# kerry-he/fsae-mpc

Hardware: AMD Instinct MI355X
Metric: QP solves/sec (batched LTV-MPC, N=40 nx=5 nu=2 fp64) (higher is better)
Workload: dtype f64

## Files before the change

### fsae-mpc_amd/_lib.py

```python
import ctypes as C
import os

_HERE = os.path.dirname(os.path.abspath(__file__))
LIB_PATH = os.environ.get("FSAEMPC_LIB") or os.path.join(_HERE, "lib", "libfsaempc.so")

EXPORTS = [
    "fsaempc_qp_default_opts", "fsaempc_qp_workspace_bytes", "fsaempc_qp_solve_batch_device", "fsaempc_qp_solve_batch",
    "fsaempc_ltv_nx", "fsaempc_ltv_nV", "fsaempc_ltv_nC", "fsaempc_ltv_build_qp_batch_device",
    "fsaempc_ltv_workspace_bytes", "fsaempc_ltv_step_batch_device", "fsaempc_ltv_step_batch_device_aux", "fsaempc_last_error", "fsaempc_selftest_mfma", "fsaempc_selftest_lane_reduce", "fsaempc_selftest_diag_factor", "fsaempc_selftest_initial_point",
    "fsaempc_debug_set_dump", "fsaempc_qp_solve_batch_device_aux", "fsaempc_qp_set_timing", "fsaempc_qp_get_timing", "fsaempc_ltv_get_timing",
    "fsaempc_seq_init", "fsaempc_seq_hotstart", "fsaempc_seq_hotstart_matrices", "fsaempc_seq_equality", "fsaempc_seq_cleanup",
    "fsaempc_obtain_reference_batch_device", "fsaempc_reference_live_batch_device",
    "fsaempc_cl_pre_batch_device", "fsaempc_cl_plant_batch_device", "fsaempc_cl_accept_batch_device",
    "fsaempc_track_from_csv", "fsaempc_track_from_points", "fsaempc_track_free", "fsaempc_track_save", "fsaempc_track_load", "fsaempc_track_last_error",
    "fsaempc_nlp_build_qp_batch_device", "fsaempc_sqp_default_opts", "fsaempc_sqp_workspace_bytes", "fsaempc_sqp_batch_device",
    "fsaempc_sqp_get_timing", "fsaempc_qp_vjp_workspace_bytes", "fsaempc_qp_vjp_batch_device",
    "fsaempc_ltv_affine_maps_batch_device", "fsaempc_ltv_step_batch_device_lambda", "fsaempc_ltv_step_vjp_workspace_bytes",
    "fsaempc_ltv_step_vjp_batch_device",
    "fsaempc_ltv_default_params", "fsaempc_ltv_build_qp_batch_device_p", "fsaempc_ltv_step_batch_device_p",
    "fsaempc_nlp_build_qp_batch_device_p", "fsaempc_sqp_batch_device_p", "fsaempc_cl_plant_batch_device_p",
    "fsaempc_ltv_blocked_nV", "fsaempc_ltv_build_qp_batch_device_b", "fsaempc_ltv_workspace_bytes_b", "fsaempc_ltv_step_batch_device_b",
    "fsaempc_qp_workspace_bytes_s", "fsaempc_qp_solve_batch_device_s", "fsaempc_qp_layout",
    "fsaempc_plan_profile_batch_device", "fsaempc_plan_reference_batch_device", "fsaempc_cl_pre_plan_batch_device",
    "fsaempc_raceline_build_qp_device", "fsaempc_plan_line_profile_batch_device", "fsaempc_plan_raceline_workspace_bytes",
# ... 345 lines not shown
```

### fsae-mpc_amd/csrc/capi_qp.hip

```cpp
#include <mutex>
#include <vector>
#include "capi_common.h"
#include "qp_solver.h"
#include "qp_sens.h"

namespace capi __attribute__((visibility("hidden"))) {
__thread char g_err[512] = "";
std::atomic<double*> g_dump{nullptr}; std::atomic<int> g_dump_stage{0};
std::atomic<bool> g_timing{false}; hipEvent_t g_ev[3] = {nullptr, nullptr, nullptr};
hipEvent_t g_evf[2] = {nullptr, nullptr};
hipEvent_t g_evs[5] = {nullptr, nullptr, nullptr, nullptr, nullptr};
double g_sqp_ms[4] = {0, 0, 0, 0};
}
using namespace capi;

extern "C" {

const char* fsaempc_last_error(void) { return g_err; }

void fsaempc_qp_default_opts(fsaempc_qp_opts* o) {
  if (!o) return;
  o->tol = 1e-8; o->tol_loose = 1e-6; o->tol_x = 1e-7; o->inf_bound = 1e9; o->max_iter = 100; o->polish = 1;
}

// ... 313 lines not shown
  return 0;
}

static int selftest(int (*test)(char* msg, int msglen)) {
  int cnt = 0;
  hipError_t e = hipGetDeviceCount(&cnt);
  if (e != hipSuccess || cnt == 0) return fail(FSAEMPC_ERR_NODEVICE, "no HIP device");
  char msg[256] = "";
  int bad = test(msg, sizeof(msg));
  if (bad != 0) snprintf(g_err, sizeof(g_err), "%s", msg);
  return bad;
}
int fsaempc_selftest_mfma(void) { return selftest(qp_selftest_mfma); }
int fsaempc_selftest_lane_reduce(void) { return selftest(qp_selftest_lane_reduce); }
int fsaempc_selftest_diag_factor(void) { return selftest(qp_selftest_diag_factor); }
int fsaempc_selftest_initial_point(void) { return selftest(qp_selftest_initial_point); }

int fsaempc_debug_set_dump(double* out, int stage) { g_dump.store(out); g_dump_stage.store(stage); return 0; }

int fsaempc_qp_set_timing(int enable) {
  if (enable && !g_ev[0]) {
    for (hipEvent_t& ev : g_ev) if (int rc = launched(hipEventCreate(&ev), "hipEventCreate")) return rc;
    for (hipEvent_t& ev : g_evf) if (int rc = launched(hipEventCreate(&ev), "hipEventCreate")) return rc;
    for (hipEvent_t& ev : g_evs) if (int rc = launched(hipEventCreate(&ev), "hipEventCreate")) return rc;
  }
  g_timing.store(enable != 0);
  return 0;
}

int fsaempc_ltv_get_timing(double* build_ms, double* prep_ms, double* solve_ms, double* post_ms) {
// ... 31 lines not shown
```

### fsae-mpc_amd/csrc/qp_probe.h

```cpp
#pragma once
#include "qp_solve_kernel.h"

template <int T, int NB> __global__ __launch_bounds__(64) void syrk_probe_kernel(QpParams P, int reps) {
  const int b = blockIdx.x;
  extern __shared__ double lds[];
  Ctx k;
  ctx_setup<T>(k, P, b, lds);
  const QpSolveLds L = qp_solve_lds(T, NB, P.d.np);
  double* MB = lds + L.vecs;
  k.ring = MB + L.border + L.tiles; k.cof = k.ring + L.ring;
  for (int js = 0; js < k.JT; ++js) {
    const int ix = js * 64 + k.lane;
    rowp(k, R_D)[ix] = 1.0; rowp(k, R_W1)[ix] = 0.5; rowp(k, R_W2)[ix] = 0.25; rowp(k, R_W3)[ix] = 2.0;
  }
  __syncthreads();
  v4d acc[Tri<T>::NT];
  acc_init<T>(k, acc);
  const unsigned long long t0 = __builtin_amdgcn_s_memtime();
  for (int r = 0; r < reps; ++r) {
    Stream<T> st;
    st.open(k);
    pass_syrk<T, NB>(k, st, acc, vecp(k, V_P1), vecp(k, V_P2), vecp(k, V_P3), MB);
    st.close();
    __syncthreads();
  }
  const unsigned long long t1 = __builtin_amdgcn_s_memtime();
  double cs = 0;
#pragma unroll
  for (int i = 0; i < Tri<T>::NT; ++i) cs += acc[i][0] + acc[i][1] + acc[i][2] + acc[i][3];
  cs = wave_sum(cs);
  if (k.lane == 0) { P.dump[b] = (double)(t1 - t0) / reps; P.dump[gridDim.x + b] = cs; }
}

__global__ __launch_bounds__(64) void overlap_probe_kernel(double* out, int reps) {
  const double x = 1.0 + 1e-9 * threadIdx.x, y = 1e-12 * (threadIdx.x + 1);
  v4d acc[8]; double f[8];
#pragma unroll
  for (int i = 0; i < 8; ++i) { acc[i] = v4d{0.0, 0.0, 0.0, 0.0}; f[i] = 1.0 + i; }
  __builtin_amdgcn_sched_barrier(0);
  const unsigned long long t0 = __builtin_amdgcn_s_memtime();
  for (int r = 0; r < reps; ++r) {
#pragma unroll
    for (int i = 0; i < 16; ++i) acc[i & 7] = __builtin_amdgcn_mfma_f64_16x16x4f64(x, y, acc[i & 7], 0, 0, 0);
    __builtin_amdgcn_sched_barrier(0);
  }
  const unsigned long long t1 = __builtin_amdgcn_s_memtime();
  for (int r = 0; r < reps; ++r) {
#pragma unroll
    for (int i = 0; i < 32; ++i) f[i & 7] = fma(f[i & 7], x, y);
    __builtin_amdgcn_sched_barrier(0);
  }
  const unsigned long long t2 = __builtin_amdgcn_s_memtime();
  for (int r = 0; r < reps; ++r) {
#pragma unroll
    for (int i = 0; i < 16; ++i) {
      acc[i & 7] = __builtin_amdgcn_mfma_f64_16x16x4f64(x, y, acc[i & 7], 0, 0, 0);
      f[(2 * i) & 7] = fma(f[(2 * i) & 7], x, y); f[(2 * i + 1) & 7] = fma(f[(2 * i + 1) & 7], x, y);
    }
// ... 26 lines not shown
  for (int r = 0; r < reps; ++r) {
    acc_init<T>(k, acc);
#pragma unroll
    for (int K = 0; K < T; ++K) {
#pragma unroll
      for (int p = 0; p < 4; ++p) if (k.q + 4 * p == k.c) acc[Tri<T>::idx(K, K)][p] += 20.0;
    }
    for (int i = k.lane; i < 16 * T; i += 64) RV[i] = 1.0 + (i & 15);
    __syncthreads();
    __builtin_amdgcn_sched_barrier(0);
    unsigned long long t0 = __builtin_amdgcn_s_memtime();
    reg_factor<T, 1>(k, acc, YL, 1e-30);
    __builtin_amdgcn_sched_barrier(0);
    unsigned long long t1 = __builtin_amdgcn_s_memtime();
    tt[0] += t1 - t0;
    v4d Yk, none = {0.0, 0.0, 0.0, 0.0};
#pragma unroll
    for (int K = 0; K < T; ++K) {
#pragma unroll
      for (int p = 0; p < 4; ++p) { Yk[p] = (k.q + 4 * p == k.c) ? 1.0 : 0.0; if (k.q + 4 * p == k.c) acc[Tri<T>::idx(K, K)][p] += 30.0; }
      diag_factor<DiagForm<T, 1>::form>(k, acc[Tri<T>::idx(K, K)], Yk, none, 1e-30);
      cs += Yk[0];
    }
    __builtin_amdgcn_sched_barrier(0);
    unsigned long long t2 = __builtin_amdgcn_s_memtime();
    tt[1] += t2 - t1;
#pragma unroll
    for (int K = 0; K < T; ++K) { tile_store(k, YL + K * 272, acc[Tri<T>::idx(K, K)]); __syncthreads(); acc[Tri<T>::idx(K, K)] = tile_load_t(k, YL + K * 272); }
    __builtin_amdgcn_sched_barrier(0);
    unsigned long long t3 = __builtin_amdgcn_s_memtime();
    tt[2] += t3 - t2;
    double y[T][4];
    vec_forward<T, true>(k, acc, YL, RV, y);
    WAVE_SYNC();
    vec_backward<T, true>(k, acc, YL, y, RV);
    WAVE_SYNC();
// ... 10 lines not shown
```

### fsae-mpc_amd/csrc/qp_selftest.h

```cpp
#pragma once
#include <stdlib.h>
#include <stdio.h>
#include "qp_solve_kernel.h"

namespace {

__global__ void mfma_selftest_kernel(const double* Am, const double* Bm, double* Cm) {
  const int lane = threadIdx.x;
  const double a = Am[(lane & 15) * 4 + (lane >> 4)];
  const double bb = Bm[(lane >> 4) * 16 + (lane & 15)];
  v4d c = {0, 0, 0, 0};
  c = __builtin_amdgcn_mfma_f64_16x16x4f64(a, bb, c, 0, 0, 0);
#pragma unroll
  for (int p = 0; p < 4; ++p) Cm[((lane >> 4) + 4 * p) * 16 + (lane & 15)] = c[p];
}

DEVINL bool same_bits(double a, double b) { return __double_as_longlong(a) == __double_as_longlong(b) || (a != a && b != b); }
template <class OP> DEVINL double lds_grp16(double* sh, int lane, double v) {
  const int src[4] = {lane ^ 1, lane ^ 2, (lane & ~7) | (7 - (lane & 7)), (lane & ~15) | (15 - (lane & 15))};
#pragma unroll
  for (int s = 0; s < 4; ++s) {
    sh[lane] = v; __syncthreads();
    const double o = sh[src[s]]; __syncthreads();
    v = OP::f(v, o);
// ... 72 lines not shown
      double a[4] = {x[4], x[5], x[6], x[7]};
      wave_sum(a);
      int nb = 0;
#pragma unroll
      for (int i = 0; i < 4; ++i) nb += same_bits(a[i], wave_sum_zf(x[4 + i])) ? 0 : 1;
      if (nb && first < 0) first = 100 * 65;
      bad += nb;
    }
    if (bad != before && first_round < 0) first_round = r;
  }
  if (bad) {
    if (atomicAdd(&out[0], bad) == 0) { out[1] = first; out[2] = first_round; out[3] = lane; }
  }
}

template <int FORM> DEVINL int diag_factor_bad_vs_old(const Ctx& k, const v4d& U0, const v4d& R0, double floor_abs, const v4d& Uo, const v4d& Yo, const v4d& Ro, int bo) {
  v4d U = U0, R = R0, Y;
#pragma unroll
  for (int p = 0; p < 4; ++p) Y[p] = (k.q + 4 * p == k.c) ? 1.0 : 0.0;
  const int b = diag_factor<FORM>(k, U, Y, R, floor_abs);
  int bad = (b != bo) ? 1 : 0;
#pragma unroll
  for (int p = 0; p < 4; ++p)
    bad += (__double_as_longlong(U[p]) != __double_as_longlong(Uo[p])) + (__double_as_longlong(Y[p]) != __double_as_longlong(Yo[p])) +
           (__double_as_longlong(R[p]) != __double_as_longlong(Ro[p]));
  return bad;
}
__global__ __launch_bounds__(64) void diag_factor_selftest_kernel(const double* __restrict__ in, int ntiles, double floor_abs, int* __restrict__ out) {
  Ctx k = {};
  k.lane = threadIdx.x; k.c = k.lane & 15; k.q = k.lane >> 4;
  int bad = 0, first = -1, form = 0;
  for (int t = 0; t < ntiles; ++t) {
    v4d U0, R0, Uo, Ro, Yo;
#pragma unroll
    for (int p = 0; p < 4; ++p) {
      U0[p] = in[(size_t)t * 512 + (k.q + 4 * p) * 16 + k.c];
      R0[p] = in[(size_t)t * 512 + 256 + (k.q + 4 * p) * 16 + k.c];
      Yo[p] = (k.q + 4 * p == k.c) ? 1.0 : 0.0;
    }
    Uo = U0; Ro = R0;
    const int bo = diag_factor<0>(k, Uo, Yo, Ro, floor_abs);
    const int b1 = diag_factor_bad_vs_old<1>(k, U0, R0, floor_abs, Uo, Yo, Ro, bo);
    const int b2 = diag_factor_bad_vs_old<2>(k, U0, R0, floor_abs, Uo, Yo, Ro, bo);
    if ((b1 | b2) && first < 0) { first = t; form = b1 ? 1 : 2; }
    bad += b1 + b2;
  }
  if (bad) {
    if (atomicAdd(&out[0], bad) == 0) { out[1] = first; out[2] = form; out[3] = k.lane; }
  }
}

template <int T, int NB> __global__ __launch_bounds__(64) void initial_point_selftest_kernel(QpParams P, int* __restrict__ out) {
  extern __shared__ double lds[];
  Ctx k;
  (void)ctx_setup<T>(k, P, 0, lds);
  const QpSolveLds L = qp_solve_lds(T, NB, P.d.np);
  k.ring = lds + L.vecs + L.border + L.tiles;
  k.cof = k.ring + L.ring;
  const int lane = k.lane, J = k.J, JT = k.JT;
  double* Xv = vecp(k, V_X); double* P3o = vecp(k, V_P1); double* P3n = vecp(k, V_P3);
  double* W3 = rowp(k, R_W3); double* Vo = rowp(k, R_VA); double* Vn = rowp(k, R_V);
  const double* Lb = rowp(k, R_L); const double* Ub = rowp(k, R_U);
  Stream<T> st;
// ... 127 lines not shown
  }
  double* d = 0; int* dout = 0; int hout[4] = {0, 0, 0, 0};
  if (hipMalloc(&d, sizeof(double) * ntiles * 512) != hipSuccess || hipMalloc(&dout, sizeof(hout)) != hipSuccess) { free(h); if (d) (void)hipFree(d); return -1; }
  (void)hipMemcpy(d, h, sizeof(double) * ntiles * 512, hipMemcpyHostToDevice);
  (void)hipMemset(dout, 0, sizeof(hout));
  free(h);
  hipLaunchKernelGGL(diag_factor_selftest_kernel, dim3(1), dim3(64), 0, 0, d, ntiles, floor_abs, dout);
  hipError_t e = hipDeviceSynchronize();
  if (e == hipSuccess) e = hipMemcpy(hout, dout, sizeof(hout), hipMemcpyDeviceToHost);
  (void)hipFree(d); (void)hipFree(dout);
  if (e != hipSuccess) { snprintf(msg, msglen, "diag_factor selftest: %s", hipGetErrorString(e)); return -1; }
  if (hout[0]) snprintf(msg, msglen, "diag_factor forms: %d mismatches with the former form, first: tile %d form %d lane %d", hout[0], hout[1], hout[2], hout[3]);
  return hout[0];
}

template <int T, int NB> static hipError_t initial_point_launch(const QpParams& P, int* dout) {
  hipError_t e = hipFuncSetAttribute(reinterpret_cast<const void*>(&initial_point_selftest_kernel<T, NB>), hipFuncAttributeMaxDynamicSharedMemorySize, (int)P.d.lds_solve);
  if (e != hipSuccess) return e;
  hipLaunchKernelGGL((initial_point_selftest_kernel<T, NB>), dim3(1), dim3(64), P.d.lds_solve, 0, P, dout);
  return hipGetLastError();
}
static int initial_point_shape(int nV, int nC, char* msg, int msglen) {
  QpDims d;
  qp_make_dims(nV, nC, &d);
  const int nb = d.nb, ncu = nV - nb;
  const double inf = 1e20;
  const size_t nH = (size_t)nV * nV, nA = (size_t)nC * nV, nin = nH + nA + 3 * (size_t)nV + 2 * (size_t)nC;
  double* h = (double*)calloc(nin, sizeof(double));
  if (!h) return -1;
  double *H = h, *A = H + nH, *g = A + nA, *lb = g + nV, *ub = lb + nV, *lbA = ub + nV, *ubA = lbA + nC;
// ... 76 lines not shown
```

### fsae-mpc_amd/csrc/qp_solve_kernel.h

```cpp
#pragma once
#include "qp_solver.h"
#include "qp_lane.h"
#include "qp_rules.h"

#ifndef QP_SOLVE_PAIR
#define QP_SOLVE_PAIR 0
#endif
#ifndef QP_DIAG_FLAT
#define QP_DIAG_FLAT 1
#endif
#ifndef QP_SYRK_INTERLEAVE
#define QP_SYRK_INTERLEAVE 0
#endif
#ifndef QP_STARTUP_ATW
#define QP_STARTUP_ATW 0
#endif
#ifndef QP_SWEEP_BATCH
#define QP_SWEEP_BATCH 6
#endif

namespace {

template <int T> struct Tri {
  static constexpr int NT = T * (T + 1) / 2;
// ... 446 lines not shown
  v4d Z;
#pragma unroll
  for (int p = 0; p < 4; ++p) Z[p] = slot[(k.q + 4 * p) * 17 + k.c];
  return Z;
}
DEVINL v4d tile_load_t(const Ctx& k, const double* slot) {
  v4d Z;
#pragma unroll
  for (int p = 0; p < 4; ++p) Z[p] = slot[k.c * 17 + k.q + 4 * p];
  return Z;
}

DEVINL double on_lanes(unsigned long long mask, double v, double otherwise) {
  return __builtin_amdgcn_inverse_ballot_w64(mask) ? v : otherwise;
}
template <int FORM> DEVINL int diag_factor(const Ctx& k, v4d& Ud, v4d& Yk, v4d& rk, double floor_abs) {
  constexpr bool FLAT = FORM >= 1;
  int bad = 0;
#pragma unroll
  for (int p = 0; p < 4; ++p) {
    const double d00 = rl(Ud[p], 4 * p + 0), d01 = rl(Ud[p], 4 * p + 1), d02 = rl(Ud[p], 4 * p + 2), d03 = rl(Ud[p], 4 * p + 3);
    const double d11 = rl(Ud[p], 16 + 4 * p + 1), d12 = rl(Ud[p], 16 + 4 * p + 2), d13 = rl(Ud[p], 16 + 4 * p + 3);
    const double d22 = rl(Ud[p], 32 + 4 * p + 2), d23 = rl(Ud[p], 32 + 4 * p + 3);
    const double d33 = rl(Ud[p], 48 + 4 * p + 3);
    auto piv = [&](double t) {
      if constexpr (FORM >= 2) {
        const bool low = !(t > floor_abs);
        bad |= (low & !(fabs(t) < INFINITY)) ? 1 : 0;
        t = low ? floor_abs : t;
      } else {
        if (!(t > floor_abs)) { if (!(fabs(t) < INFINITY)) bad = 1; t = floor_abs; }
      }
      return rsqrt(t);
    };
    const double i0 = piv(d00);
    const double r01 = d01 * i0, r02 = d02 * i0, r03 = d03 * i0;
    const double i1 = piv(fma(-r01, r01, d11));
    const double r12 = fma(-r01, r02, d12) * i1, r13 = fma(-r01, r03, d13) * i1;
    const double i2 = piv(fma(-r12, r12, fma(-r02, r02, d22)));
    const double r23 = fma(-r12, r13, fma(-r02, r03, d23)) * i2;
    const double i3 = piv(fma(-r23, r23, fma(-r13, r13, fma(-r03, r03, d33))));
    const double w10 = -r01 * i0 * i1;
    const double w20 = -fma(r12, w10, r02 * i0) * i2, w21 = -r12 * i1 * i2;
    const double w30 = -fma(r23, w20, fma(r13, w10, r03 * i0)) * i3, w31 = -fma(r23, w21, r13 * i1) * i3, w32 = -r23 * i2 * i3;
    const v4d z = {0.0, 0.0, 0.0, 0.0};
    if constexpr (FLAT) {
      const unsigned long long L0 = 1ull << (4 * p), L1 = 1ull << (16 + 4 * p), L2 = 1ull << (32 + 4 * p), L3 = 1ull << (48 + 4 * p);
      double wa = on_lanes(L0, i0, 0.0);
      wa = on_lanes(L0 << 1, w10, wa); wa = on_lanes(L0 << 2, w20, wa); wa = on_lanes(L0 << 3, w30, wa);
      wa = on_lanes(L1 << 1, i1, wa); wa = on_lanes(L1 << 2, w21, wa); wa = on_lanes(L1 << 3, w31, wa);
      wa = on_lanes(L2 << 2, i2, wa); wa = on_lanes(L2 << 3, w32, wa);
      wa = on_lanes(L3 << 3, i3, wa);
      const v4d nu = __builtin_amdgcn_mfma_f64_16x16x4f64(wa, Ud[p], z, 0, 0, 0);
      Ud[p] = nu[p];
      double a = 0.0;
      if (p < 3) {
        a = on_lanes(0x0001000100010001ull * (0xFFFFull & (0xFFFFull << (4 * p + 4))), -Ud[p], 0.0);
        Ud = __builtin_amdgcn_mfma_f64_16x16x4f64(a, Ud[p], Ud, 0, 0, 0);
      }
      const v4d ny = __builtin_amdgcn_mfma_f64_16x16x4f64(wa, Yk[p], z, 0, 0, 0);
      const v4d nr = __builtin_amdgcn_mfma_f64_16x16x4f64(wa, rk[p], z, 0, 0, 0);
      Yk[p] = ny[p]; rk[p] = nr[p];
      if (p < 3) {
        Yk = __builtin_amdgcn_mfma_f64_16x16x4f64(a, Yk[p], Yk, 0, 0, 0);
        rk = __builtin_amdgcn_mfma_f64_16x16x4f64(a, rk[p], rk, 0, 0, 0);
      }
      if constexpr (FORM >= 2) asm("" : "+v"(bad));
    } else {
      const int a_ = k.c - 4 * p;
      double wa = 0.0;
      if (k.q == 0) wa = a_ == 0 ? i0 : (a_ == 1 ? w10 : (a_ == 2 ? w20 : (a_ == 3 ? w30 : 0.0)));
      if (k.q == 1) wa = a_ == 1 ? i1 : (a_ == 2 ? w21 : (a_ == 3 ? w31 : 0.0));
      if (k.q == 2) wa = a_ == 2 ? i2 : (a_ == 3 ? w32 : 0.0);
      if (k.q == 3) wa = a_ == 3 ? i3 : 0.0;
      const v4d nu = __builtin_amdgcn_mfma_f64_16x16x4f64(wa, Ud[p], z, 0, 0, 0);
      const v4d ny = __builtin_amdgcn_mfma_f64_16x16x4f64(wa, Yk[p], z, 0, 0, 0);
      const v4d nr = __builtin_amdgcn_mfma_f64_16x16x4f64(wa, rk[p], z, 0, 0, 0);
      Ud[p] = nu[p]; Yk[p] = ny[p]; rk[p] = nr[p];
      if (p < 3) {
        const double a = (k.c > 4 * p + 3) ? -Ud[p] : 0.0;
        Yk = __builtin_amdgcn_mfma_f64_16x16x4f64(a, Yk[p], Yk, 0, 0, 0);
        rk = __builtin_amdgcn_mfma_f64_16x16x4f64(a, rk[p], rk, 0, 0, 0);
        Ud = __builtin_amdgcn_mfma_f64_16x16x4f64(a, Ud[p], Ud, 0, 0, 0);
      }
    }
  }
#pragma unroll
  for (int p = 0; p < 4; ++p) if (k.c < k.q + 4 * p) Ud[p] = 0.0;
  return bad;
}

template <int T, int NB> struct DiagForm { static constexpr int form = (T == 5 && NB > 0) ? QP_DIAG_FLAT : 0; };

template <int T, int NB> struct SweepBatch { static constexpr int nsb = (T == 5 && NB > 0) ? QP_SWEEP_BATCH : 2; };

template <int T, int NB, int K> struct FactorStep {
  static DEVINL int run(const Ctx& k, v4d* acc, double* YL, double floor_abs) {
    v4d Yk, none = {0.0, 0.0, 0.0, 0.0};
#pragma unroll
    for (int p = 0; p < 4; ++p) Yk[p] = (k.q + 4 * p == k.c) ? 1.0 : 0.0;
    int bad = diag_factor<DiagForm<T, NB>::form>(k, acc[Tri<T>::idx(K, K)], Yk, none, floor_abs);
    tile_store(k, YL + K * 272, Yk);
    WAVE_SYNC();
    const v4d Wk = tile_load_t(k, YL + K * 272);
    const v4d& UKK = acc[Tri<T>::idx(K, K)];
#pragma unroll
    for (int Jt = K + 1; Jt < T; ++Jt) {
      v4d Rr = acc[Tri<T>::idx(K, Jt)];
      v4d Ukj = mfma4_new(Wk, Rr);
      mfma4_sub<T>(UKK, Ukj, Rr);
#pragma unroll
      for (int p = 0; p < 4; ++p) Ukj = __builtin_amdgcn_mfma_f64_16x16x4f64(Wk[p], Rr[p], Ukj, 0, 0, 0);
      acc[Tri<T>::idx(K, Jt)] = Ukj;
    }
#pragma unroll
    for (int I = K + 1; I < T; ++I) {
      const v4d& UKI = acc[Tri<T>::idx(K, I)];
#pragma unroll
      for (int Jt = I; Jt < T; ++Jt) mfma4_sub<T>(UKI, acc[Tri<T>::idx(K, Jt)], acc[Tri<T>::idx(I, Jt)]);
    }
    return bad | FactorStep<T, NB, K + 1>::run(k, acc, YL, floor_abs);
  }
};
template <int T, int NB> struct FactorStep<T, NB, T> {
  static DEVINL int run(const Ctx&, v4d*, double*, double) { return 0; }
};
template <int T, int NB> DEVINL int reg_factor(const Ctx& k, v4d* acc, double* YL, double floor_abs) {
  return FactorStep<T, NB, 0>::run(k, acc, YL, floor_abs);
}

template <int T, bool REFINE, int NV> DEVINL void vec_forward(const Ctx& k, const v4d* acc, const double* YL, const double* const (&B)[NV], double (&y)[NV][T][4]) {
#pragma unroll
  for (int K = 0; K < T; ++K) {
    double s[NV], t[NV];
#pragma unroll
    for (int v = 0; v < NV; ++v) {
      s[v] = 0.0;
#pragma unroll
      for (int I = 0; I < K; ++I)
#pragma unroll
        for (int p = 0; p < 4; ++p) s[v] = fma(acc[Tri<T>::idx(I, K)][p], y[v][I][p], s[v]);
    }
    if (K > 0) q_sum(s);
// ... 1031 lines not shown
```

### fsae-mpc_amd/csrc/qp_solver.h

```cpp
#pragma once
#include <hip/hip_runtime.h>
#include <stddef.h>

#define QP_MAX_T 12
#ifndef QP_WG_W
#define QP_WG_W 8
#endif
#define QP_BREAKDOWN_TRY_TOL 1e-4

enum RowArr { R_L = 0, R_U, R_TL, R_TU, R_ZL, R_ZU, R_V, R_D, R_W1, R_W2, R_W3, R_VA, R_VC, R_RPL, R_RPU, R_CB1, R_CC1, R_CB2, R_CC2, R_NARR };

struct QpDims {
  int n, m;
  int T, np;
  int nb, NB, nc;
  int Kq, ntr;
  int prep_tw;
  int J, JB;
  int nu;
  int rowlen;
  size_t off_Aw, off_meta, off_Hw, off_gw, off_E, off_F, off_Ab, off_Hb, off_rows, off_save, off_bad, ws_per_qp;
  size_t lds_solve, lds_prep;
  int W;
  int NBk;
// ... 18 lines not shown
  const int* score_in;
  int* order;
};
#define QP_ORDER_MIN_BATCH 256
inline size_t qp_order_bytes(int batch) { return batch > QP_ORDER_MIN_BATCH ? (((size_t)2 * batch * sizeof(int)) + 255) & ~(size_t)255 : 0; }

#define QP_NO_SLACK_HINT (-1)
void qp_make_dims(int n, int m, QpDims* d, int n_slack = QP_NO_SLACK_HINT);
__host__ __device__ inline int qp_user_index(const QpDims& d, int i) { const int ncu = d.nu - d.nb; return i < ncu ? i : (i >= d.nc && d.nb > 0 ? ncu + (i - d.nc) : (i < d.nu && d.nb == 0 ? i : -1)); }
__host__ __device__ inline int qp_solver_index(const QpDims& d, int u) { const int ncu = d.nu - d.nb; return (d.nb > 0 && u >= ncu) ? d.nc + (u - ncu) : u; }
bool qp_runs_wavefront_kernel(const QpDims& d);
hipError_t qp_launch(const QpParams& P, int batch, hipStream_t st, hipEvent_t ev_mid = nullptr);
int qp_selftest_mfma(char* msg, int msglen);
int qp_selftest_lane_reduce(char* msg, int msglen);
int qp_selftest_diag_factor(char* msg, int msglen);
int qp_selftest_initial_point(char* msg, int msglen);
#define QP_SOLVE_NVEC 10
#define QP_SOLVE_RING(T) (3 * (T))
struct QpSolveLds {
  size_t vecs, border, tiles, ring, cof;
  __host__ __device__ size_t total() const { return vecs + border + tiles + ring + cof; }
};
__host__ __device__ inline QpSolveLds qp_solve_lds(int T, int NB, int np) {
  return {(size_t)QP_SOLVE_NVEC * np, (size_t)(NB > 0 ? NB : 1) * np, (size_t)T * 272, (size_t)QP_SOLVE_RING(T) * 128, (size_t)(6 + NB) * 64};
}
#define QP_WG_NVEC_FIXED 14
inline size_t qp_wg_lds_base_bytes(const QpDims& d, int W, int NBk) {
  const size_t part2 = (size_t)W * d.np;
  const size_t extra = (size_t)240 * d.T > part2 ? (size_t)240 * d.T : part2;
  return ((size_t)(QP_WG_NVEC_FIXED + 2 * NBk) * d.np + (size_t)d.T * 272 + (size_t)d.T * 256 + 256 + (size_t)W * 96 +
// ... 4 lines not shown
```

### fsae-mpc_amd/csrc/qp_solver.hip

```cpp
#include <hip/hip_runtime.h>
#include <math.h>
#include <stdint.h>
#include <stdlib.h>
#include <stdio.h>
#include "qp_solver.h"
#include "qp_lane.h"

#if !defined(QP_TU) || QP_TU == 0
#define QP_MAIN_TU 1
#else
#define QP_MAIN_TU 0
#endif
#include "qp_solve_kernel.h"

#if QP_MAIN_TU
namespace {

#ifdef QP_PREP_STAMPS
#define PSTAMP(id) do { __builtin_amdgcn_sched_barrier(0); const unsigned long long t_ = __builtin_amdgcn_s_memtime(); pst[id] += t_ - pst_t0; pst_t0 = t_; __builtin_amdgcn_sched_barrier(0); } while (0)
#else
#define PSTAMP(id) do { } while (0)
#endif
__global__ __launch_bounds__(1024) void qp_prep_kernel(QpParams P) {
  const int b = blockIdx.x, tid = threadIdx.x, w = tid >> 6, lane = tid & 63, c = lane & 15, q = lane >> 4;
// ... 464 lines not shown
  if (P.order) {
    hipLaunchKernelGGL(qp_order_kernel, dim3(1), dim3(1024), 0, st, P.score, P.order, batch);
    e = hipGetLastError();
    if (e != hipSuccess) return e;
  }
  if (ev_mid) { e = hipEventRecord(ev_mid, st); if (e != hipSuccess) return e; }
#ifdef QP_PROBE
  if (P.dump && P.dump_stage == 7 && P.d.T == 5) {
    (void)hipFuncSetAttribute(reinterpret_cast<const void*>(&factor_probe_kernel<5>), hipFuncAttributeMaxDynamicSharedMemorySize, (int)P.d.lds_solve);
    hipLaunchKernelGGL((factor_probe_kernel<5>), dim3(batch), dim3(64), P.d.lds_solve, st, P, 8);
    return hipGetLastError();
  }
  if (P.dump && P.dump_stage == 8 && P.d.T == 5 && P.d.NB == 1) {
    (void)hipFuncSetAttribute(reinterpret_cast<const void*>(&syrk_probe_kernel<5, 1>), hipFuncAttributeMaxDynamicSharedMemorySize, (int)P.d.lds_solve);
    hipLaunchKernelGGL((syrk_probe_kernel<5, 1>), dim3(batch), dim3(64), P.d.lds_solve, st, P, 16);
    hipLaunchKernelGGL(overlap_probe_kernel, dim3(batch), dim3(64), 0, st, P.dump + 2 * (size_t)batch, 2048);
    return hipGetLastError();
  }
#endif
  if (!qp_runs_wavefront_kernel(P.d)) return qp_wg_launch(P, batch, st);
#if !defined(QP_TU)
  switch (P.d.T) {
#if defined(QP_ONLY_T)
    case QP_ONLY_T: return launch_solve_T<QP_ONLY_T>(P, batch, st);
#else
    case 1: return launch_solve_T<1>(P, batch, st);
    case 2: return launch_solve_T<2>(P, batch, st);
    case 3: return launch_solve_T<3>(P, batch, st);
    case 4: return launch_solve_T<4>(P, batch, st);
    case 5: return launch_solve_T<5>(P, batch, st);
    case 6: return launch_solve_T<6>(P, batch, st);
// ... 17 lines not shown
```

### include/fsaempc.h

```cpp
#ifndef FSAEMPC_H
#define FSAEMPC_H

#ifdef __cplusplus
extern "C" {
#endif

#define FSAEMPC_ERR_ARG      (-1)
#define FSAEMPC_ERR_DIM      (-2)
#define FSAEMPC_ERR_HIP      (-3)
#define FSAEMPC_ERR_NODEVICE (-4)
#define FSAEMPC_ERR_WORKSPACE (-5)
#define FSAEMPC_ERR_SOLVER   (-6)

#define FSAEMPC_MAX_NV 196

#define FSAEMPC_MODEL_KINEMATIC 0
#define FSAEMPC_MODEL_DYNAMIC   1

typedef struct {
  double tol;
  double tol_loose;
  double tol_x;
  double inf_bound;
  int    max_iter;
// ... 514 lines not shown
} fsaempc_track;

int fsaempc_track_from_csv(const char* path, int M, fsaempc_track* out);
int fsaempc_track_from_points(const double* x, const double* y, int n, int M, fsaempc_track* out);
void fsaempc_track_free(fsaempc_track* t);
int fsaempc_track_save(const fsaempc_track* t, const char* path);
int fsaempc_track_load(const char* path, fsaempc_track* out);
int fsaempc_track_cones_from_csv(const char* path, double** left, int* n_left, double** right, int* n_right);
void fsaempc_track_cones_free(double* cones);
const char* fsaempc_track_last_error(void);

const char* fsaempc_last_error(void);
int fsaempc_selftest_mfma(void);
int fsaempc_selftest_lane_reduce(void);
int fsaempc_selftest_diag_factor(void);
int fsaempc_selftest_initial_point(void);
int fsaempc_debug_set_dump(double* out, int stage);

int fsaempc_qp_set_timing(int enable);
int fsaempc_qp_get_timing(double* prep_ms, double* solve_ms);
int fsaempc_ltv_get_timing(double* build_ms, double* prep_ms, double* solve_ms, double* post_ms);

#ifdef __cplusplus
}
#endif
#endif
```

Measured before the change: 442,300.

## Add look-ahead blocked Cholesky that interleaves trailing updates into diagonal factor

Adds an optional look-ahead mode to the register-tiled blocked Cholesky factor. The next diagonal block is updated first, and the remaining trailing-matrix MFMA updates are deferred and spread across the scalar pivot points of the next diagonal factorization, so matrix work can overlap the serial rsqrt/fma chain. It also removes the unused rk right-hand-side MFMAs from diag_factor, and adds a bitwise-equivalence selftest plus probe tweaks. The look-ahead defaults to off (QP_FACTOR_AHEAD=0), so by default only the dropped dead MFMAs change the hot path.

```diff
diff --git a/fsae-mpc_amd/_lib.py b/fsae-mpc_amd/_lib.py
--- a/fsae-mpc_amd/_lib.py
+++ b/fsae-mpc_amd/_lib.py
@@ -7,7 +7,7 @@
 EXPORTS = [
     "fsaempc_qp_default_opts", "fsaempc_qp_workspace_bytes", "fsaempc_qp_solve_batch_device", "fsaempc_qp_solve_batch",
     "fsaempc_ltv_nx", "fsaempc_ltv_nV", "fsaempc_ltv_nC", "fsaempc_ltv_build_qp_batch_device",
-    "fsaempc_ltv_workspace_bytes", "fsaempc_ltv_step_batch_device", "fsaempc_ltv_step_batch_device_aux", "fsaempc_last_error", "fsaempc_selftest_mfma", "fsaempc_selftest_lane_reduce", "fsaempc_selftest_diag_factor", "fsaempc_selftest_initial_point",
+    "fsaempc_ltv_workspace_bytes", "fsaempc_ltv_step_batch_device", "fsaempc_ltv_step_batch_device_aux", "fsaempc_last_error", "fsaempc_selftest_mfma", "fsaempc_selftest_lane_reduce", "fsaempc_selftest_diag_factor", "fsaempc_selftest_factor_ahead", "fsaempc_selftest_initial_point",
     "fsaempc_debug_set_dump", "fsaempc_qp_solve_batch_device_aux", "fsaempc_qp_set_timing", "fsaempc_qp_get_timing", "fsaempc_ltv_get_timing",
     "fsaempc_seq_init", "fsaempc_seq_hotstart", "fsaempc_seq_hotstart_matrices", "fsaempc_seq_equality", "fsaempc_seq_cleanup",
     "fsaempc_obtain_reference_batch_device", "fsaempc_reference_live_batch_device",
diff --git a/fsae-mpc_amd/csrc/capi_qp.hip b/fsae-mpc_amd/csrc/capi_qp.hip
--- a/fsae-mpc_amd/csrc/capi_qp.hip
+++ b/fsae-mpc_amd/csrc/capi_qp.hip
@@ -351,6 +351,7 @@
 int fsaempc_selftest_mfma(void) { return selftest(qp_selftest_mfma); }
 int fsaempc_selftest_lane_reduce(void) { return selftest(qp_selftest_lane_reduce); }
 int fsaempc_selftest_diag_factor(void) { return selftest(qp_selftest_diag_factor); }
+int fsaempc_selftest_factor_ahead(void) { return selftest(qp_selftest_factor_ahead); }
 int fsaempc_selftest_initial_point(void) { return selftest(qp_selftest_initial_point); }
 
 int fsaempc_debug_set_dump(double* out, int stage) { g_dump.store(out); g_dump_stage.store(stage); return 0; }
diff --git a/fsae-mpc_amd/csrc/qp_probe.h b/fsae-mpc_amd/csrc/qp_probe.h
--- a/fsae-mpc_amd/csrc/qp_probe.h
+++ b/fsae-mpc_amd/csrc/qp_probe.h
@@ -37,11 +37,15 @@
   v4d acc[8]; double f[8];
 #pragma unroll
   for (int i = 0; i < 8; ++i) { acc[i] = v4d{0.0, 0.0, 0.0, 0.0}; f[i] = 1.0 + i; }
+#pragma unroll
+  for (int i = 0; i < 8; ++i) asm volatile("" : "+a"(acc[i]));
   __builtin_amdgcn_sched_barrier(0);
   const unsigned long long t0 = __builtin_amdgcn_s_memtime();
   for (int r = 0; r < reps; ++r) {
 #pragma unroll
     for (int i = 0; i < 16; ++i) acc[i & 7] = __builtin_amdgcn_mfma_f64_16x16x4f64(x, y, acc[i & 7], 0, 0, 0);
+#pragma unroll
+    for (int i = 0; i < 8; ++i) asm volatile("" : "+a"(acc[i]));
     __builtin_amdgcn_sched_barrier(0);
   }
   const unsigned long long t1 = __builtin_amdgcn_s_memtime();
@@ -98,12 +102,12 @@
     __builtin_amdgcn_sched_barrier(0);
     unsigned long long t1 = __builtin_amdgcn_s_memtime();
     tt[0] += t1 - t0;
-    v4d Yk, none = {0.0, 0.0, 0.0, 0.0};
+    v4d Yk;
 #pragma unroll
     for (int K = 0; K < T; ++K) {
 #pragma unroll
       for (int p = 0; p < 4; ++p) { Yk[p] = (k.q + 4 * p == k.c) ? 1.0 : 0.0; if (k.q + 4 * p == k.c) acc[Tri<T>::idx(K, K)][p] += 30.0; }
-      diag_factor<DiagForm<T, 1>::form>(k, acc[Tri<T>::idx(K, K)], Yk, none, 1e-30);
+      diag_factor<DiagForm<T, 1>::form>(k, acc[Tri<T>::idx(K, K)], Yk, 1e-30);
       cs += Yk[0];
     }
     __builtin_amdgcn_sched_barrier(0);
diff --git a/fsae-mpc_amd/csrc/qp_selftest.h b/fsae-mpc_amd/csrc/qp_selftest.h
--- a/fsae-mpc_amd/csrc/qp_selftest.h
+++ b/fsae-mpc_amd/csrc/qp_selftest.h
@@ -110,16 +110,15 @@
   }
 }
 
-template <int FORM> DEVINL int diag_factor_bad_vs_old(const Ctx& k, const v4d& U0, const v4d& R0, double floor_abs, const v4d& Uo, const v4d& Yo, const v4d& Ro, int bo) {
-  v4d U = U0, R = R0, Y;
+template <int FORM> DEVINL int diag_factor_bad_vs_old(const Ctx& k, const v4d& U0, double floor_abs, const v4d& Uo, const v4d& Yo, int bo) {
+  v4d U = U0, Y;
 #pragma unroll
   for (int p = 0; p < 4; ++p) Y[p] = (k.q + 4 * p == k.c) ? 1.0 : 0.0;
-  const int b = diag_factor<FORM>(k, U, Y, R, floor_abs);
+  const int b = diag_factor<FORM>(k, U, Y, floor_abs);
   int bad = (b != bo) ? 1 : 0;
 #pragma unroll
   for (int p = 0; p < 4; ++p)
-    bad += (__double_as_longlong(U[p]) != __double_as_longlong(Uo[p])) + (__double_as_longlong(Y[p]) != __double_as_longlong(Yo[p])) +
-           (__double_as_longlong(R[p]) != __double_as_longlong(Ro[p]));
+    bad += (__double_as_longlong(U[p]) != __double_as_longlong(Uo[p])) + (__double_as_longlong(Y[p]) != __double_as_longlong(Yo[p]));
   return bad;
 }
 __global__ __launch_bounds__(64) void diag_factor_selftest_kernel(const double* __restrict__ in, int ntiles, double floor_abs, int* __restrict__ out) {
@@ -127,22 +126,74 @@
   k.lane = threadIdx.x; k.c = k.lane & 15; k.q = k.lane >> 4;
   int bad = 0, first = -1, form = 0;
   for (int t = 0; t < ntiles; ++t) {
-    v4d U0, R0, Uo, Ro, Yo;
+    v4d U0, Uo, Yo;
 #pragma unroll
     for (int p = 0; p < 4; ++p) {
       U0[p] = in[(size_t)t * 512 + (k.q + 4 * p) * 16 + k.c];
-      R0[p] = in[(size_t)t * 512 + 256 + (k.q + 4 * p) * 16 + k.c];
       Yo[p] = (k.q + 4 * p == k.c) ? 1.0 : 0.0;
     }
-    Uo = U0; Ro = R0;
-    const int bo = diag_factor<0>(k, Uo, Yo, Ro, floor_abs);
-    const int b1 = diag_factor_bad_vs_old<1>(k, U0, R0, floor_abs, Uo, Yo, Ro, bo);
-    const int b2 = diag_factor_bad_vs_old<2>(k, U0, R0, floor_abs, Uo, Yo, Ro, bo);
+    Uo = U0;
+    const int bo = diag_factor<0>(k, Uo, Yo, floor_abs);
+    const int b1 = diag_factor_bad_vs_old<1>(k, U0, floor_abs, Uo, Yo, bo);
+    const int b2 = diag_factor_bad_vs_old<2>(k, U0, floor_abs, Uo, Yo, bo);
     if ((b1 | b2) && first < 0) { first = t; form = b1 ? 1 : 2; }
     bad += b1 + b2;
   }
   if (bad) {
     if (atomicAdd(&out[0], bad) == 0) { out[1] = first; out[2] = form; out[3] = k.lane; }
+  }
+}
+
+template <int MODE> DEVINL int factor_ahead_bad_vs_old(const Ctx& k, const double* __restrict__ M, double* YL, double floor_abs, const double* Ao, const double* YLo, int bo) {
+  constexpr int T = 5;
+  v4d A[Tri<T>::NT];
+#pragma unroll
+  for (int I = 0; I < T; ++I)
+#pragma unroll
+    for (int Jt = I; Jt < T; ++Jt)
+#pragma unroll
+      for (int p = 0; p < 4; ++p) A[Tri<T>::idx(I, Jt)][p] = M[(size_t)(16 * I + k.q + 4 * p) * 80 + 16 * Jt + k.c];
+  WAVE_SYNC();
+  const int b = reg_factor<T, 1, MODE>(k, A, YL, floor_abs);
+  WAVE_SYNC();
+  int bad = (b != bo) ? 1 : 0;
+#pragma unroll
+  for (int t = 0; t < Tri<T>::NT; ++t)
+#pragma unroll
+    for (int p = 0; p < 4; ++p) bad += same_bits(A[t][p], Ao[(t * 4 + p) * 64 + k.lane]) ? 0 : 1;
+  for (int i = k.lane; i < T * 272; i += 64)
+    if ((i % 17) < 16) bad += same_bits(YL[i], YLo[i]) ? 0 : 1;
+  return bad;
+}
+__global__ __launch_bounds__(64) void factor_ahead_selftest_kernel(const double* __restrict__ in, int nmat, double floor_abs, double* ref, int* __restrict__ out) {
+  constexpr int T = 5;
+  __shared__ double YLo[T * 272], YLn[T * 272];
+  Ctx k = {};
+  k.lane = threadIdx.x; k.c = k.lane & 15; k.q = k.lane >> 4;
+  for (int i = k.lane; i < T * 272; i += 64) { YLo[i] = 0.0; YLn[i] = 0.0; }
+  int bad = 0, first = -1, mode = 0;
+  for (int t = 0; t < nmat; ++t) {
+    const double* M = in + (size_t)t * 6400;
+    v4d Ao[Tri<T>::NT];
+#pragma unroll
+    for (int I = 0; I < T; ++I)
+#pragma unroll
+      for (int Jt = I; Jt < T; ++Jt)
+#pragma unroll
+        for (int p = 0; p < 4; ++p) Ao[Tri<T>::idx(I, Jt)][p] = M[(size_t)(16 * I + k.q + 4 * p) * 80 + 16 * Jt + k.c];
+    WAVE_SYNC();
+    const int bo = reg_factor<T, 1, 0>(k, Ao, YLo, floor_abs);
+#pragma unroll
+    for (int i = 0; i < Tri<T>::NT; ++i)
+#pragma unroll
+      for (int p = 0; p < 4; ++p) ref[(i * 4 + p) * 64 + k.lane] = Ao[i][p];
+    const int b1 = factor_ahead_bad_vs_old<1>(k, M, YLn, floor_abs, ref, YLo, bo);
+    const int b2 = factor_ahead_bad_vs_old<2>(k, M, YLn, floor_abs, ref, YLo, bo);
+    if ((b1 | b2) && first < 0) { first = t; mode = b1 ? 1 : 2; }
+    bad += b1 + b2;
+  }
+  if (bad) {
+    if (atomicAdd(&out[0], bad) == 0) { out[1] = first; out[2] = mode; out[3] = k.lane; }
   }
 }
 
@@ -300,6 +351,54 @@
   return hout[0];
 }
 
+int qp_selftest_factor_ahead(char* msg, int msglen) {
+  const int nmat = 64, n = 80;
+  const double floor_abs = 1e-9;
+  double* h = (double*)malloc(sizeof(double) * nmat * n * n);
+  double* Q = (double*)malloc(sizeof(double) * n * n);
+  if (!h || !Q) { free(h); free(Q); return -1; }
+  unsigned long long st = 0xA0761D6478BD642Full;
+  auto rnd = [&]() { st = st * 6364136223846793005ull + 1442695040888963407ull; return ((unsigned)(st >> 33)) / 2147483648.0; };
+  for (int t = 0; t < nmat; ++t) {
+    double* D = h + (size_t)t * n * n;
+    double sv[80], v[80];
+    for (int i = 0; i < n; ++i) for (int j = 0; j < n; ++j) Q[i * n + j] = i == j ? 1.0 : 0.0;
+    for (int r = 0; r < 3; ++r) {
+      double vv = 0;
+      for (int i = 0; i < n; ++i) { v[i] = 2.0 * rnd() - 1.0; vv += v[i] * v[i]; }
+      for (int i = 0; i < n; ++i) {
+        double qv = 0;
+        for (int j = 0; j < n; ++j) qv += Q[i * n + j] * v[j];
+        for (int j = 0; j < n; ++j) Q[i * n + j] -= 2.0 * qv * v[j] / vv;
+      }
+    }
+    const double lc = 10.0 * (t < 61 ? t / 60.0 : 0.3);
+    for (int i = 0; i < n; ++i) sv[i] = pow(10.0, -lc * i / (n - 1.0));
+    for (int i = 0; i < n; ++i) for (int j = i; j < n; ++j) {
+      double a = 0;
+      for (int l = 0; l < n; ++l) a += Q[i * n + l] * sv[l] * Q[j * n + l];
+      D[i * n + j] = a; D[j * n + i] = a;
+    }
+    if (t == 61) for (int j = 0; j < n; ++j) { D[38 * n + j] *= 1e-6; D[j * n + 38] *= 1e-6; }
+    if (t == 62) { D[5 * n + 40] = NAN; D[40 * n + 5] = NAN; }
+    if (t == 63) D[42 * n + 42] = INFINITY;
+  }
+  free(Q);
+  double *d = 0, *dref = 0; int* dout = 0; int hout[4] = {0, 0, 0, 0};
+  if (hipMalloc(&d, sizeof(double) * nmat * n * n) != hipSuccess || hipMalloc(&dref, sizeof(double) * 15 * 4 * 64) != hipSuccess ||
+      hipMalloc(&dout, sizeof(hout)) != hipSuccess) { free(h); if (d) (void)hipFree(d); if (dref) (void)hipFree(dref); return -1; }
+  (void)hipMemcpy(d, h, sizeof(double) * nmat * n * n, hipMemcpyHostToDevice);
+  (void)hipMemset(dout, 0, sizeof(hout));
+  free(h);
+  hipLaunchKernelGGL(factor_ahead_selftest_kernel, dim3(1), dim3(64), 0, 0, d, nmat, floor_abs, dref, dout);
+  hipError_t e = hipDeviceSynchronize();
+  if (e == hipSuccess) e = hipMemcpy(hout, dout, sizeof(hout), hipMemcpyDeviceToHost);
+  (void)hipFree(d); (void)hipFree(dref); (void)hipFree(dout);
+  if (e != hipSuccess) { snprintf(msg, msglen, "factor look-ahead selftest: %s", hipGetErrorString(e)); return -1; }
+  if (hout[0]) snprintf(msg, msglen, "factor look-ahead: %d mismatches with the former order, first: matrix %d mode %d lane %d", hout[0], hout[1], hout[2], hout[3]);
+  return hout[0];
+}
+
 template <int T, int NB> static hipError_t initial_point_launch(const QpParams& P, int* dout) {
   hipError_t e = hipFuncSetAttribute(reinterpret_cast<const void*>(&initial_point_selftest_kernel<T, NB>), hipFuncAttributeMaxDynamicSharedMemorySize, (int)P.d.lds_solve);
   if (e != hipSuccess) return e;
diff --git a/fsae-mpc_amd/csrc/qp_solve_kernel.h b/fsae-mpc_amd/csrc/qp_solve_kernel.h
--- a/fsae-mpc_amd/csrc/qp_solve_kernel.h
+++ b/fsae-mpc_amd/csrc/qp_solve_kernel.h
@@ -8,6 +8,12 @@
 #endif
 #ifndef QP_DIAG_FLAT
 #define QP_DIAG_FLAT 1
+#endif
+#ifndef QP_FACTOR_AHEAD
+#define QP_FACTOR_AHEAD 0
+#endif
+#ifndef QP_FACTOR_SHARE_MAX
+#define QP_FACTOR_SHARE_MAX 11
 #endif
 #ifndef QP_SYRK_INTERLEAVE
 #define QP_SYRK_INTERLEAVE 0
@@ -484,7 +490,12 @@
 DEVINL double on_lanes(unsigned long long mask, double v, double otherwise) {
   return __builtin_amdgcn_inverse_ballot_w64(mask) ? v : otherwise;
 }
-template <int FORM> DEVINL int diag_factor(const Ctx& k, v4d& Ud, v4d& Yk, v4d& rk, double floor_abs) {
+struct NoDefer {
+  DEVINL void point(int, int) {}
+  DEVINL void rest() {}
+};
+constexpr int QP_FACTOR_POINTS = 7;
+template <int FORM, class Defer = NoDefer> DEVINL int diag_factor(const Ctx& k, v4d& Ud, v4d& Yk, double floor_abs, Defer&& defer = Defer{}) {
   constexpr bool FLAT = FORM >= 1;
   int bad = 0;
 #pragma unroll
@@ -503,22 +514,29 @@
       }
       return rsqrt(t);
     };
+    defer.point(p, 0);
     const double i0 = piv(d00);
     const double r01 = d01 * i0, r02 = d02 * i0, r03 = d03 * i0;
+    defer.point(p, 1);
     const double i1 = piv(fma(-r01, r01, d11));
     const double r12 = fma(-r01, r02, d12) * i1, r13 = fma(-r01, r03, d13) * i1;
+    defer.point(p, 2);
     const double i2 = piv(fma(-r12, r12, fma(-r02, r02, d22)));
     const double r23 = fma(-r12, r13, fma(-r02, r03, d23)) * i2;
+    defer.point(p, 3);
     const double i3 = piv(fma(-r23, r23, fma(-r13, r13, fma(-r03, r03, d33))));
+    defer.point(p, 4);
     const double w10 = -r01 * i0 * i1;
     const double w20 = -fma(r12, w10, r02 * i0) * i2, w21 = -r12 * i1 * i2;
     const double w30 = -fma(r23, w20, fma(r13, w10, r03 * i0)) * i3, w31 = -fma(r23, w21, r13 * i1) * i3, w32 = -r23 * i2 * i3;
+    defer.point(p, 5);
     const v4d z = {0.0, 0.0, 0.0, 0.0};
     if constexpr (FLAT) {
       const unsigned long long L0 = 1ull << (4 * p), L1 = 1ull << (16 + 4 * p), L2 = 1ull << (32 + 4 * p), L3 = 1ull << (48 + 4 * p);
       double wa = on_lanes(L0, i0, 0.0);
       wa = on_lanes(L0 << 1, w10, wa); wa = on_lanes(L0 << 2, w20, wa); wa = on_lanes(L0 << 3, w30, wa);
       wa = on_lanes(L1 << 1, i1, wa); wa = on_lanes(L1 << 2, w21, wa); wa = on_lanes(L1 << 3, w31, wa);
+      defer.point(p, 6);
       wa = on_lanes(L2 << 2, i2, wa); wa = on_lanes(L2 << 3, w32, wa);
       wa = on_lanes(L3 << 3, i3, wa);
       const v4d nu = __builtin_amdgcn_mfma_f64_16x16x4f64(wa, Ud[p], z, 0, 0, 0);
@@ -529,14 +547,11 @@
         Ud = __builtin_amdgcn_mfma_f64_16x16x4f64(a, Ud[p], Ud, 0, 0, 0);
       }
       const v4d ny = __builtin_amdgcn_mfma_f64_16x16x4f64(wa, Yk[p], z, 0, 0, 0);
-      const v4d nr = __builtin_amdgcn_mfma_f64_16x16x4f64(wa, rk[p], z, 0, 0, 0);
-      Yk[p] = ny[p]; rk[p] = nr[p];
-      if (p < 3) {
-        Yk = __builtin_amdgcn_mfma_f64_16x16x4f64(a, Yk[p], Yk, 0, 0, 0);
-        rk = __builtin_amdgcn_mfma_f64_16x16x4f64(a, rk[p], rk, 0, 0, 0);
-      }
+      Yk[p] = ny[p];
+      if (p < 3) Yk = __builtin_amdgcn_mfma_f64_16x16x4f64(a, Yk[p], Yk, 0, 0, 0);
       if constexpr (FORM >= 2) asm("" : "+v"(bad));
     } else {
+      defer.point(p, 6);
       const int a_ = k.c - 4 * p;
       double wa = 0.0;
       if (k.q == 0) wa = a_ == 0 ? i0 : (a_ == 1 ? w10 : (a_ == 2 ? w20 : (a_ == 3 ? w30 : 0.0)));
@@ -545,16 +560,15 @@
       if (k.q == 3) wa = a_ == 3 ? i3 : 0.0;
       const v4d nu = __builtin_amdgcn_mfma_f64_16x16x4f64(wa, Ud[p], z, 0, 0, 0);
       const v4d ny = __builtin_amdgcn_mfma_f64_16x16x4f64(wa, Yk[p], z, 0, 0, 0);
-      const v4d nr = __builtin_amdgcn_mfma_f64_16x16x4f64(wa, rk[p], z, 0, 0, 0);
-      Ud[p] = nu[p]; Yk[p] = ny[p]; rk[p] = nr[p];
+      Ud[p] = nu[p]; Yk[p] = ny[p];
       if (p < 3) {
         const double a = (k.c > 4 * p + 3) ? -Ud[p] : 0.0;
         Yk = __builtin_amdgcn_mfma_f64_16x16x4f64(a, Yk[p], Yk, 0, 0, 0);
-        rk = __builtin_amdgcn_mfma_f64_16x16x4f64(a, rk[p], rk, 0, 0, 0);
         Ud = __builtin_amdgcn_mfma_f64_16x16x4f64(a, Ud[p], Ud, 0, 0, 0);
       }
     }
   }
+  defer.rest();
 #pragma unroll
   for (int p = 0; p < 4; ++p) if (k.c < k.q + 4 * p) Ud[p] = 0.0;
   return bad;
@@ -564,14 +578,83 @@
 
 template <int T, int NB> struct SweepBatch { static constexpr int nsb = (T == 5 && NB > 0) ? QP_SWEEP_BATCH : 2; };
 
-template <int T, int NB, int K> struct FactorStep {
-  static DEVINL int run(const Ctx& k, v4d* acc, double* YL, double floor_abs) {
-    v4d Yk, none = {0.0, 0.0, 0.0, 0.0};
+template <int T, int NB> struct FactorAhead { static constexpr int mode = (T == 5 && NB > 0) ? QP_FACTOR_AHEAD : 0; };
+
+DEVINL void block_row_mfma(int i, const v4d& Wk, const v4d& UKK, v4d& Mkj, v4d& Ukj) {
+  const v4d z = {0.0, 0.0, 0.0, 0.0};
+  const int p = i & 3;
+  if (i < 4) Ukj = __builtin_amdgcn_mfma_f64_16x16x4f64(Wk[p], Mkj[p], p == 0 ? z : Ukj, 0, 0, 0);
+  else if (i < 8) Mkj = __builtin_amdgcn_mfma_f64_16x16x4f64(-UKK[p], Ukj[p], Mkj, 0, 0, 0);
+  else {
+    Ukj = __builtin_amdgcn_mfma_f64_16x16x4f64(Wk[p], Mkj[p], Ukj, 0, 0, 0);
+    if (p == 3) Mkj = Ukj;
+  }
+}
+
+template <int T, int K, int MODE> struct FactorDefer {
+  static constexpr int R = T - K - 2 > 0 ? T - K - 2 : 0;
+  static constexpr int NTRAIL = R > 0 ? (T - K - 1) * (T - K) / 2 - 1 : 0;
+  static constexpr int N = 12 * R + 4 * NTRAIL;
+  static constexpr int SHARE = (N + 3) / 4 < QP_FACTOR_SHARE_MAX ? (N + 3) / 4 : QP_FACTOR_SHARE_MAX;
+  v4d* acc;
+  v4d Wk;
+  v4d ukj[R > 0 ? R : 1];
+  DEVINL void issue(int lo, int hi) {
+    if (lo >= hi) return;
+    __builtin_amdgcn_sched_barrier(0);
+    int i = 0;
+#pragma unroll
+    for (int Jt = K + 2; Jt < T; ++Jt)
+#pragma unroll
+      for (int j = 0; j < 12; ++j, ++i)
+        if (i >= lo && i < hi) block_row_mfma(j, Wk, acc[Tri<T>::idx(K, K)], acc[Tri<T>::idx(K, Jt)], ukj[Jt - K - 2]);
+#pragma unroll
+    for (int I = K + 1; I < T; ++I)
+#pragma unroll
+      for (int Jt = I; Jt < T; ++Jt) {
+        if (I == K + 1 && Jt == K + 1) continue;
+#pragma unroll
+        for (int p = 0; p < 4; ++p, ++i)
+          if (i >= lo && i < hi)
+            acc[Tri<T>::idx(I, Jt)] = __builtin_amdgcn_mfma_f64_16x16x4f64(-acc[Tri<T>::idx(K, I)][p], acc[Tri<T>::idx(K, Jt)][p], acc[Tri<T>::idx(I, Jt)], 0, 0, 0);
+      }
+    __builtin_amdgcn_sched_barrier(0);
+  }
+  DEVINL void point(int p, int j) {
+    if constexpr (N > 0) {
+      const int lo = p * SHARE, hi = lo + SHARE < N ? lo + SHARE : N;
+      if (MODE == 1) { if (j == 0) issue(lo, hi); }
+      else {
+        const int a = lo + (j * SHARE) / QP_FACTOR_POINTS, b = lo + ((j + 1) * SHARE) / QP_FACTOR_POINTS;
+        issue(a, b < hi ? b : hi);
+      }
+    }
+  }
+  DEVINL void rest() {
+    if constexpr (N > 0) issue(4 * SHARE, N);
+  }
+};
+
+template <int T, int NB, int K, int AHEAD> struct FactorStep {
+  template <class Prev> static DEVINL int run(const Ctx& k, v4d* acc, double* YL, double floor_abs, Prev&& prev) {
+    v4d Yk;
 #pragma unroll
     for (int p = 0; p < 4; ++p) Yk[p] = (k.q + 4 * p == k.c) ? 1.0 : 0.0;
-    int bad = diag_factor<DiagForm<T, NB>::form>(k, acc[Tri<T>::idx(K, K)], Yk, none, floor_abs);
+    int bad = diag_factor<DiagForm<T, NB>::form>(k, acc[Tri<T>::idx(K, K)], Yk, floor_abs, prev);
     tile_store(k, YL + K * 272, Yk);
     WAVE_SYNC();
+    if constexpr (AHEAD != 0 && K + 1 < T) {
+      FactorDefer<T, K, AHEAD> rest;
+      rest.acc = acc;
+      rest.Wk = tile_load_t(k, YL + K * 272);
+      {
+        v4d Ukj;
+#pragma unroll
+        for (int j = 0; j < 12; ++j) block_row_mfma(j, rest.Wk, acc[Tri<T>::idx(K, K)], acc[Tri<T>::idx(K, K + 1)], Ukj);
+        mfma4_sub<T>(acc[Tri<T>::idx(K, K + 1)], acc[Tri<T>::idx(K, K + 1)], acc[Tri<T>::idx(K + 1, K + 1)]);
+      }
+      return bad | FactorStep<T, NB, K + 1, AHEAD>::run(k, acc, YL, floor_abs, rest);
+    }
     const v4d Wk = tile_load_t(k, YL + K * 272);
     const v4d& UKK = acc[Tri<T>::idx(K, K)];
 #pragma unroll
@@ -589,14 +672,14 @@
 #pragma unroll
       for (int Jt = I; Jt < T; ++Jt) mfma4_sub<T>(UKI, acc[Tri<T>::idx(K, Jt)], acc[Tri<T>::idx(I, Jt)]);
     }
-    return bad | FactorStep<T, NB, K + 1>::run(k, acc, YL, floor_abs);
+    return bad | FactorStep<T, NB, K + 1, AHEAD>::run(k, acc, YL, floor_abs, NoDefer{});
   }
 };
-template <int T, int NB> struct FactorStep<T, NB, T> {
-  static DEVINL int run(const Ctx&, v4d*, double*, double) { return 0; }
+template <int T, int NB, int AHEAD> struct FactorStep<T, NB, T, AHEAD> {
+  template <class Prev> static DEVINL int run(const Ctx&, v4d*, double*, double, Prev&&) { return 0; }
 };
-template <int T, int NB> DEVINL int reg_factor(const Ctx& k, v4d* acc, double* YL, double floor_abs) {
-  return FactorStep<T, NB, 0>::run(k, acc, YL, floor_abs);
+template <int T, int NB, int AHEAD = FactorAhead<T, NB>::mode> DEVINL int reg_factor(const Ctx& k, v4d* acc, double* YL, double floor_abs) {
+  return FactorStep<T, NB, 0, AHEAD>::run(k, acc, YL, floor_abs, NoDefer{});
 }
 
 template <int T, bool REFINE, int NV> DEVINL void vec_forward(const Ctx& k, const v4d* acc, const double* YL, const double* const (&B)[NV], double (&y)[NV][T][4]) {
diff --git a/fsae-mpc_amd/csrc/qp_solver.h b/fsae-mpc_amd/csrc/qp_solver.h
--- a/fsae-mpc_amd/csrc/qp_solver.h
+++ b/fsae-mpc_amd/csrc/qp_solver.h
@@ -56,6 +56,7 @@
 int qp_selftest_mfma(char* msg, int msglen);
 int qp_selftest_lane_reduce(char* msg, int msglen);
 int qp_selftest_diag_factor(char* msg, int msglen);
+int qp_selftest_factor_ahead(char* msg, int msglen);
 int qp_selftest_initial_point(char* msg, int msglen);
 #define QP_SOLVE_NVEC 10
 #define QP_SOLVE_RING(T) (3 * (T))
diff --git a/fsae-mpc_amd/csrc/qp_solver.hip b/fsae-mpc_amd/csrc/qp_solver.hip
--- a/fsae-mpc_amd/csrc/qp_solver.hip
+++ b/fsae-mpc_amd/csrc/qp_solver.hip
@@ -502,7 +502,8 @@
   if (P.dump && P.dump_stage == 8 && P.d.T == 5 && P.d.NB == 1) {
     (void)hipFuncSetAttribute(reinterpret_cast<const void*>(&syrk_probe_kernel<5, 1>), hipFuncAttributeMaxDynamicSharedMemorySize, (int)P.d.lds_solve);
     hipLaunchKernelGGL((syrk_probe_kernel<5, 1>), dim3(batch), dim3(64), P.d.lds_solve, st, P, 16);
-    hipLaunchKernelGGL(overlap_probe_kernel, dim3(batch), dim3(64), 0, st, P.dump + 2 * (size_t)batch, 2048);
+    (void)hipFuncSetAttribute(reinterpret_cast<const void*>(&overlap_probe_kernel), hipFuncAttributeMaxDynamicSharedMemorySize, (int)P.d.lds_solve);
+    hipLaunchKernelGGL(overlap_probe_kernel, dim3(batch), dim3(64), P.d.lds_solve, st, P.dump + 2 * (size_t)batch, 2048);
     return hipGetLastError();
   }
 #endif
diff --git a/include/fsaempc.h b/include/fsaempc.h
--- a/include/fsaempc.h
+++ b/include/fsaempc.h
@@ -552,6 +552,7 @@
 int fsaempc_selftest_mfma(void);
 int fsaempc_selftest_lane_reduce(void);
 int fsaempc_selftest_diag_factor(void);
+int fsaempc_selftest_factor_ahead(void);
 int fsaempc_selftest_initial_point(void);
 int fsaempc_debug_set_dump(double* out, int stage);
 
```

New measurement: 441,300. Within noise of the previous version (-0.2%).
